# ShijieZhou-UCLA/feature-3dgs

Measured on NVIDIA B200. Metric: views/sec fwd+bwd @1M Gaussians/1080p/feat_dim=128, higher is better.
Workload: dtype f32

## Files before the change

feature-3dgs_b200/csrc/api.cu:

```cuda
#include <cub/cub.cuh>

#include <cstdio>
#include <cstdlib>
#include <cstring>
#include <mutex>
#include <string>
#include <vector>

#include "../../include/f3dgs_b200.h"
#include "kernels.h"

#ifndef F3DGS_FBWD_TC_DEFAULT
#define F3DGS_FBWD_TC_DEFAULT 0
#endif
#ifndef F3DGS_BWD2_DEFAULT
#define F3DGS_BWD2_DEFAULT 1
#endif
#ifndef F3DGS_TC_DEFAULT
#define F3DGS_TC_DEFAULT 1
#endif

namespace f3dgs {
std::atomic<unsigned long long> g_launches{0};
}
// ... 66 lines not shown
    size_t final_T, n_contrib, ranges, counters, bytes;
    ImgLayout(size_t HW, size_t tiles) {
        size_t o = 0;
        final_T = o;    o = align_up(o + HW * 4);
        n_contrib = o;  o = align_up(o + HW * 4);
        ranges = o;     o = align_up(o + tiles * 8);
        counters = o;   o = align_up(o + 256);
        bytes = o;
    }
};
struct BinLayout {
    size_t point_list, keys, point_list_unsorted, keys_unsorted, fixed_bytes;
    explicit BinLayout(size_t R) {
        size_t o = 0;
        point_list = o;           o = align_up(o + R * 4);
        keys = o;                 o = align_up(o + R * 8);
        point_list_unsorted = o;  o = align_up(o + R * 4);
        keys_unsorted = o;        o = align_up(o + R * 8);
        fixed_bytes = o;
    }
};

struct ListLayout {
    size_t w, meta, cnt, bytes;
    ListLayout(size_t R, size_t tiles) {
        size_t o = 0;
        w = o;     o = align_up(o + 8 * R * 32 * sizeof(float));
        meta = o;  o = align_up(o + 8 * R * sizeof(uint2));
        cnt = o;   o = align_up(o + 8 * tiles * sizeof(uint32_t));
        bytes = o;
    }
};

inline bool bwd2_mode() {
    static int on = -1;
    if (on < 0) {
        const char* e = getenv("F3DGS_BWD2");
        on = e ? (e[0] == '1' ? 1 : 0) : F3DGS_BWD2_DEFAULT;
    }
    return on != 0;
}

inline bool tc_mode(int C, const float* features) {
    static int on = -1;
    if (on < 0) {
        const char* e = getenv("F3DGS_TC");
        on = e ? (e[0] == '1' ? 1 : 0) : F3DGS_TC_DEFAULT;
    }
    static int min_c = -1;
    if (min_c < 0) {
        const char* e = getenv("F3DGS_TC_MIN_C");
// ... 292 lines not shown
            char* lists = nullptr;
            const ListLayout ll((size_t)R, tiles);
            if (C > 0 && R > 0) {
                static std::once_flag once;
                std::call_once(once, [] {
                    int dev = 0;
                    cudaGetDevice(&dev);
                    cudaMemPool_t pool;
                    if (cudaDeviceGetDefaultMemPool(&pool, dev) == cudaSuccess) {
                        unsigned long long keep = ~0ull;
                        cudaMemPoolSetAttribute(pool, cudaMemPoolAttrReleaseThreshold, &keep);
                    }
                });
                cudaError_t ea = cudaMallocAsync((void**)&lists, ll.bytes, stream);
                if (ea != cudaSuccess)
                    return fail(F3DGS_ERR_ALLOC, w + ": cudaMallocAsync of " + std::to_string(ll.bytes) +
                                                     " bytes for the backward instance lists failed: " +
                                                     cudaGetErrorString(ea));
            }
            e = launch_composite_bwd_geom_slim(
                vg, ranges, point_list, rec, background, final_T, n_contrib, dL_dpix, dL_depths, dL_dmean2D, dL_dconic,
                dL_dopacity, dL_dcolor, dL_dz, counters + 16, stream, lists ? reinterpret_cast<float*>(lists + ll.w) : nullptr,
                lists ? reinterpret_cast<uint2*>(lists + ll.meta) : nullptr,
                lists ? reinterpret_cast<uint32_t*>(lists + ll.cnt) : nullptr);
            if (e == cudaSuccess && lists)
                e = launch_feature_bwd(vp, ranges, reinterpret_cast<const float*>(lists + ll.w),
                                       reinterpret_cast<const uint2*>(lists + ll.meta),
                                       reinterpret_cast<const uint32_t*>(lists + ll.cnt), dL_dfeaturepix,
                                       dL_dsemantic_feature, counters + 48, stream, fbwd_tc_mode(C));
            if (lists) cudaFreeAsync(lists, stream);
        } else {
            e = launch_composite_bwd(vp, ranges, point_list, rec, background, final_T, n_contrib, dL_dpix,
                                     dL_dfeaturepix, dL_depths, dL_dmean2D, dL_dconic, dL_dopacity, dL_dcolor,
                                     dL_dsemantic_feature, dL_dz, counters + 16, stream);
        }
    }
    if (e != cudaSuccess) return fail(F3DGS_ERR_CUDA, std::string("composite_bwd launch: ") + cudaGetErrorString(e));
    STAGE_CHECK("composite_bwd");
    if (composite_done) CUDA_TRY(cudaEventRecord(composite_done, stream));
    {
        StageTimer t(F3DGS_STAGE_PREPROCESS_BWD, stream);
        launch_preprocess_bwd(vp, means3D, radii, shs, clamped, scales, rotations, cov3d, dL_dmean2D, dL_dconic,
                              dL_dmean3D, dL_dcolor, dL_dcov3D, dL_dsh, dL_dscale, dL_drot, dL_dz, stream, accumulate,
                              grad_accum, denom);
    }
    STAGE_CHECK("preprocess_bwd");
    return 0;
}

}

// ... 102 lines not shown
```

feature-3dgs_b200/csrc/composite_bwd.cu:

```cuda
#include <cstdio>
#include <cstdlib>

#include "composite_common.cuh"

namespace f3dgs {

#ifndef F3DGS_TIMING_BUILD
#define F3DGS_TIMING_BUILD 0
#endif
#ifndef F3DGS_DIAG_NO_FEAT_RED
#define F3DGS_DIAG_NO_FEAT_RED 0
#endif
#ifndef F3DGS_DIAG_NO_FMA
#define F3DGS_DIAG_NO_FMA 0
#endif
#ifndef F3DGS_DIAG_NO_GEOM_RED
#define F3DGS_DIAG_NO_GEOM_RED 0
#endif
static constexpr bool kTimingB = F3DGS_TIMING_BUILD != 0;
#define BTICK() ((kTimingB && args.dbg) ? clock64() : 0ll)

#ifndef F3DGS_PAIR_SKIP
#define F3DGS_PAIR_SKIP 1
#endif
// ... 30 lines not shown
    uint32_t red_gid[kBlocksPerTile][kRedSlots];
};
using BwdSmem = BwdSmemT<RingV2<0>>;

struct BwdArgs {
    ProducerArgs pa;
    const float* bg;
    const float* final_T;
    const uint32_t* n_contrib;
    const float* dL_dpix;
    const float* dL_dfeat_pix;
    const float* dL_ddepth;
    float* dL_dmean2D;
    float* dL_dconic;
    float* dL_dopacity;
    float* dL_dcolor;
    float* dL_dfeature;
    float* dL_dz;
    int vec_io;
    long long* dbg;
    float* list_w;
    uint2* list_meta;
    uint32_t* list_cnt;
};

__device__ __forceinline__ float* geom_dst(const BwdArgs& args, int v, uint32_t gid) {
    switch (v) {
        case 0: return args.dL_dmean2D + 3 * (size_t)gid;
        case 1: return args.dL_dmean2D + 3 * (size_t)gid + 1;
        case 2: return args.dL_dconic + 4 * (size_t)gid;
        case 3: return args.dL_dconic + 4 * (size_t)gid + 1;
        case 4: return args.dL_dconic + 4 * (size_t)gid + 3;
        case 5: return args.dL_dopacity + gid;
        case 6: return args.dL_dz + gid;
        default: return args.dL_dcolor + 3 * (size_t)gid + (v - 7);
    }
}


template <int CH, int BPA, bool SLIM = false, bool EMIT = false>
__global__ void __launch_bounds__(SLIM ? (kAlphaWarp0 + Layout<BPA>::kAlphaWarps) * 32 : Layout<BPA>::kThreads, SLIM ? kSlimCtas : 1)
composite_bwd_kernel(const BwdArgs args) {
    static_assert(!SLIM || CH == 0, "the slim layout has no feature warps");
    extern __shared__ __align__(128) unsigned char smem_raw[];
    using RING = typename RingSelect<0, SLIM>::type;
    using SMEM = BwdSmemT<RING>;
// ... 201 lines not shown
                                const float dL_dG = r1.w * dL_dalpha;
                                const float gdx = Gs * dx, gdy = Gs * dy;
                                const float dG_ddelx = -gdx * r1.x - gdy * r1.y;
                                const float dG_ddely = -gdy * r1.z - gdx * r1.y;
                                v[0] = dL_dG * dG_ddelx * ddelx_dx;
                                v[1] = dL_dG * dG_ddely * ddely_dy;
                                v[2] = -0.5f * gdx * dx * dL_dG;
                                v[3] = -0.5f * gdx * dy * dL_dG;
                                v[4] = -0.5f * gdy * dy * dL_dG;
                                v[5] = Gs * dL_dalpha;
                                v[6] = wgt * p.dLd;
                            }
                            const uint32_t pm = __ballot_sync(0xffffffffu, contrib);
                            if (pm) {
                                if (kTimingB) nA_pm++;
                                if (CH > 0) {
                                    ws->w[k][lane] = wgt;
                                    if (lane == 0) ws->pm[k] = pm;
                                    km |= 1u << k;
                                }
                                if (EMIT) {
                                    const size_t e = ebase[bi] + ecount[bi];
                                    args.list_w[e * 32 + lane] = wgt;
                                    if (lane == 0) args.list_meta[e] = make_uint2(st.gid[k], pm);
                                    ecount[bi]++;
                                }
                                if (do_geom) {
#pragma unroll
                                    for (int i = 0; i < kRedVals; i++) red[i * kRedSlots + nslots][lane] = v[i];
                                    if (lane == 0) red_gid[nslots] = st.gid[k];
                                    nslots++;
                                    if (nslots == kRedSlots) flush();
                                }
                            }
                        }
                    }
                }
                if (CH > 0) {
                    __syncwarp();
                    if (lane == 0) {
                        ws->km = km;
                        ws->last = last;
                        ws->first = first;
                        ws->work = work;
                        mbar_arrive(&ring.wfull[b][j]);
                    }
                }
// ... 231 lines not shown
    g_launches++;
    if (timing) {
        static long long host[256 * 32 * 8];
        cudaMemcpyAsync(host, dbg, sizeof(host), cudaMemcpyDeviceToHost, s);
        cudaStreamSynchronize(s);
        const int nA = Layout<BPA>::kAlphaWarps, f0 = Layout<BPA>::kFeatWarp0;
        double A[6] = {0, 0, 0, 0, 0, 0}, F[6] = {0, 0, 0, 0, 0, 0};
        for (int c = 0; c < grid; c++) {
            for (int w = 0; w < nA; w++) for (int i = 0; i < 6; i++) A[i] += host[(c * 32 + kAlphaWarp0 + w) * 8 + i];
            for (int w = 0; w < 8; w++) for (int i = 0; i < 6; i++) F[i] += host[(c * 32 + f0 + w) * 8 + i];
        }
        fprintf(stderr, "[f3dgs timing bwd CH=%d BPA=%d] per-warp mean cycles: alpha total %.0f wait_full %.0f wait_wempty %.0f flush %.0f hits %.0f pm %.0f | feature total %.0f wait_wfull %.0f wait_full %.0f tile_load %.0f k %.0f k_loop %.0f\n",
                CH, BPA, A[0] / (grid * nA), A[1] / (grid * nA), A[2] / (grid * nA), A[3] / (grid * nA), A[4] / (grid * nA),
                A[5] / (grid * nA), F[0] / (grid * 8), F[1] / (grid * 8), F[2] / (grid * 8), F[3] / (grid * 8), F[4] / (grid * 8), F[5] / (grid * 8));
    }
    return cudaGetLastError();
}

cudaError_t launch_composite_bwd_geom_slim(const ViewParams& vp, const uint2* ranges, const uint32_t* point_list,
                                           const SplatRec* rec, const float* bg, const float* final_T,
                                           const uint32_t* n_contrib, const float* dL_dpix, const float* dL_ddepth,
                                           float* dL_dmean2D, float* dL_dconic, float* dL_dopacity, float* dL_dcolor,
                                           float* dL_dz, int* work_counter, cudaStream_t s, float* list_w,
                                           uint2* list_meta, uint32_t* list_cnt) {
    using SMEM = BwdSmemT<RingSlim>;
    const bool emit = list_w != nullptr;
    const size_t smem = sizeof(SMEM);
    static std::atomic<int> sms_of_device[64];
    int dev = 0;
    cudaGetDevice(&dev);
    if (dev < 0 || dev >= 64) return cudaErrorInvalidDevice;
    if (sms_of_device[dev].load() == 0) {
        cudaError_t e = cudaFuncSetAttribute(composite_bwd_kernel<0, 1, true>, cudaFuncAttributeMaxDynamicSharedMemorySize,
                                             (int)smem);
        if (e == cudaSuccess)
            e = cudaFuncSetAttribute(composite_bwd_kernel<0, 1, true, true>, cudaFuncAttributeMaxDynamicSharedMemorySize,
                                     (int)smem);
        if (e != cudaSuccess) return e;
        int n = 0;
        cudaDeviceGetAttribute(&n, cudaDevAttrMultiProcessorCount, dev);
        sms_of_device[dev].store(n > 0 ? n : 148);
    }
    BwdArgs a;
    a.pa.ranges = ranges; a.pa.point_list = point_list; a.pa.rec = rec; a.pa.features = nullptr;
    a.pa.n_contrib = n_contrib; a.pa.work_counter = work_counter;
    a.pa.W = vp.W; a.pa.H = vp.H; a.pa.C = 0;
    a.pa.tiles_x = (int)vp.grid_x; a.pa.num_tiles = (int)(vp.grid_x * vp.grid_y); a.pa.chunks = 1; a.pa.use_bulk = 0;
    a.bg = bg; a.final_T = final_T; a.n_contrib = n_contrib; a.dL_dpix = dL_dpix; a.dL_dfeat_pix = nullptr;
    a.dL_ddepth = dL_ddepth; a.dL_dmean2D = dL_dmean2D; a.dL_dconic = dL_dconic; a.dL_dopacity = dL_dopacity;
    a.dL_dcolor = dL_dcolor; a.dL_dfeature = nullptr; a.dL_dz = dL_dz; a.vec_io = 0; a.dbg = nullptr;
    a.list_w = list_w; a.list_meta = list_meta; a.list_cnt = list_cnt;
    cudaError_t e = cudaMemsetAsync(work_counter, 0, sizeof(int), s);
    if (e != cudaSuccess) return e;
    const int grid = min(a.pa.num_tiles, kSlimCtas * sms_of_device[dev].load());
    if (emit)
        composite_bwd_kernel<0, 1, true, true><<<grid, (kAlphaWarp0 + Layout<1>::kAlphaWarps) * 32, smem, s>>>(a);
    else
        composite_bwd_kernel<0, 1, true><<<grid, (kAlphaWarp0 + Layout<1>::kAlphaWarps) * 32, smem, s>>>(a);
    g_launches++;
    return cudaGetLastError();
}

#define F3DGS_BWD_DISPATCH(CHV) launch_bwd_t<CHV, 1>(vp, a, s)

cudaError_t launch_composite_bwd(const ViewParams& vp, const uint2* ranges, const uint32_t* point_list,
                                 const SplatRec* rec, const float* bg, const float* final_T,
                                 const uint32_t* n_contrib, const float* dL_dpix, const float* dL_dfeat_pix,
                                 const float* dL_ddepth, float* dL_dmean2D, float* dL_dconic,
                                 float* dL_dopacity, float* dL_dcolor, float* dL_dfeature, float* dL_dz,
                                 int* work_counter, cudaStream_t s) {
    BwdArgs a;
    a.pa.ranges = ranges; a.pa.point_list = point_list; a.pa.rec = rec; a.pa.features = nullptr;
    a.pa.n_contrib = n_contrib; a.pa.work_counter = work_counter;
    a.pa.W = vp.W; a.pa.H = vp.H; a.pa.C = vp.C;
    a.pa.tiles_x = (int)vp.grid_x; a.pa.num_tiles = (int)(vp.grid_x * vp.grid_y); a.pa.chunks = 1;
    a.pa.use_bulk = 0;
    a.bg = bg; a.final_T = final_T; a.n_contrib = n_contrib; a.dL_dpix = dL_dpix; a.dL_dfeat_pix = dL_dfeat_pix;
    a.dL_ddepth = dL_ddepth; a.dL_dmean2D = dL_dmean2D; a.dL_dconic = dL_dconic; a.dL_dopacity = dL_dopacity;
    a.dL_dcolor = dL_dcolor; a.dL_dfeature = dL_dfeature; a.dL_dz = dL_dz; a.vec_io = 0; a.dbg = nullptr;
    a.list_w = nullptr; a.list_meta = nullptr; a.list_cnt = nullptr;
    if (vp.C == 0) return F3DGS_BWD_DISPATCH(0);
    if (vp.C <= 32) return F3DGS_BWD_DISPATCH(32);
    if (vp.C <= 64) return F3DGS_BWD_DISPATCH(64);
    return F3DGS_BWD_DISPATCH(128);
}

}
```

feature-3dgs_b200/csrc/feature_bwd.cu:

```cuda
#include <cstdio>
#include <cstdlib>

#include "composite_common.cuh"
#include "tc_common.cuh"

namespace f3dgs {

#ifndef F3DGS_LIST_CHUNK
#define F3DGS_LIST_CHUNK 16
#endif
constexpr int kListChunk = F3DGS_LIST_CHUNK;
constexpr int kFeatWarps = 4;

template <int CH, bool WITH_ROWS>
struct alignas(128) FeatSmem {
    float w[2][kListChunk][32];
};

struct FeatArgs {
    const uint2* ranges;
    const float* list_w;
    const uint2* list_meta;
    const uint32_t* list_cnt;
    const float* dL_dfeat_pix;
    float* dL_dfeature;
    int* work_counter;
    int W, H, C, tiles_x, num_tiles, chunks;
    int vec;
};

__device__ __forceinline__ void cp_async16(void* dst_smem, const void* src_gmem) {
    asm volatile("cp.async.ca.shared.global [%0], [%1], 16;" ::"r"(smem_u32(dst_smem)), "l"(src_gmem) : "memory");
}
__device__ __forceinline__ void cp_async_commit() { asm volatile("cp.async.commit_group;" ::: "memory"); }
template <int N>
__device__ __forceinline__ void cp_async_wait() {
    asm volatile("cp.async.wait_group %0;" ::"n"(N) : "memory");
}

struct ItemPos {
    int tile, chunk, b, bx0, by0;
};
__device__ __forceinline__ ItemPos decode_item(int item, const FeatArgs& a) {
    ItemPos p;
    p.b = item & (kBlocksPerTile - 1);
    const int tc = item / kBlocksPerTile;
    p.chunk = tc % a.chunks;
    p.tile = tc / a.chunks;
    const int tile_x = p.tile % a.tiles_x, tile_y = p.tile / a.tiles_x;
    p.bx0 = tile_x * 16 + (p.b & 1) * 8;
    p.by0 = tile_y * 16 + (p.b >> 1) * 4;
    return p;
}

template <int CH>
__global__ void __launch_bounds__(kFeatWarps * 32, 3) feature_bwd_kernel(const FeatArgs a) {
    extern __shared__ __align__(128) unsigned char smem_raw[];
    const int warp = __shfl_sync(0xffffffffu, threadIdx.x >> 5, 0), lane = threadIdx.x & 31;
    FeatSmem<CH, false>& sm = reinterpret_cast<FeatSmem<CH, false>*>(smem_raw)[warp];
    constexpr int LPR = CH / 4;
    constexpr int G = 32 / LPR;
    constexpr int NQ = 8 / G;
    const int grp = lane / LPR, cl = lane % LPR;
    const int W = a.W, H = a.H, C = a.C;
    const size_t HW = (size_t)H * W;

    const int items = a.num_tiles * a.chunks * kBlocksPerTile;
    for (;;) {
        int item = 0;
        if (lane == 0) item = atomicAdd(a.work_counter, 1);
        item = __shfl_sync(0xffffffffu, item, 0);
        if (item >= items) break;
        const ItemPos ip = decode_item(item, a);
        const uint32_t rx = __shfl_sync(0xffffffffu, a.ranges[ip.tile].x, 0);
        const uint32_t ry = __shfl_sync(0xffffffffu, a.ranges[ip.tile].y, 0);
        const size_t base = 8 * (size_t)rx + (size_t)ip.b * (ry - rx);
        const uint32_t n = __shfl_sync(0xffffffffu, a.list_cnt[(size_t)ip.tile * kBlocksPerTile + ip.b], 0);
        if (n == 0) continue;
        const int ch0 = ip.chunk * CH + cl * 4;
        const uint32_t nch = (n + kListChunk - 1) / kListChunk;

        auto load_meta = [&](uint32_t c) -> uint2 {
            const uint32_t e = c * kListChunk + lane;
            return (lane < kListChunk && e < n) ? __ldg(&a.list_meta[base + e]) : make_uint2(0u, 0u);
        };
        auto issue = [&](uint32_t c, int buf) {
            const uint32_t cnt = min((uint32_t)kListChunk, n - c * kListChunk);
            const float* wsrc = a.list_w + (base + (size_t)c * kListChunk) * 32;
            for (uint32_t j = lane; j < cnt * 8; j += 32) cp_async16(&sm.w[buf][0][0] + j * 4, wsrc + j * 4);
            cp_async_commit();
        };
        uint2 m_cur = load_meta(0);
        issue(0, 0);

        float2 dO2[NQ][2][4];
#define DOB(q, i, c) (((i) & 1) ? dO2[q][(i) >> 1][c].y : dO2[q][(i) >> 1][c].x)
#pragma unroll
        for (int q = 0; q < NQ; q++)
#pragma unroll
            for (int r = 0; r < 2; r++)
#pragma unroll
                for (int c = 0; c < 4; c++) dO2[q][r][c] = make_float2(0.f, 0.f);
#pragma unroll
        for (int c = 0; c < 4; c++) {
            const int ch = ch0 + c;
            if (ch >= C) continue;
            const float* plane = a.dL_dfeat_pix + (size_t)ch * HW;
            if (G == 1 && (a.vec & 2)) {
#pragma unroll
                for (int y = 0; y < 4; y++) {
                    const int yy = ip.by0 + y;
                    if (yy >= H) continue;
#pragma unroll
                    for (int half = 0; half < 2; half++) {
                        const int xx = ip.bx0 + half * 4;
                        if (xx >= W) continue;
                        const int qa = (y >> 1) * 4 + half * 2, i0 = (y & 1) * 2;
                        const float4 v = ld_nc_f4(plane + (size_t)yy * W + xx);
                        DOB(qa % NQ, i0, c) = v.x;
                        DOB(qa % NQ, i0 + 1, c) = v.y;
                        DOB((qa + 1) % NQ, i0, c) = v.z;
                        DOB((qa + 1) % NQ, i0 + 1, c) = v.w;
                    }
                }
            } else {
#pragma unroll
                for (int qi = 0; qi < NQ; qi++) {
                    const int q = qi * G + grp;
#pragma unroll
                    for (int i = 0; i < 4; i++) {
                        const int xx = ip.bx0 + (q & 3) * 2 + (i & 1), yy = ip.by0 + (q >> 2) * 2 + (i >> 1);
                        if (xx < W && yy < H) DOB(qi, i, c) = __ldg(plane + (size_t)yy * W + xx);
                    }
                }
            }
        }
#undef DOB

        for (uint32_t c = 0; c < nch; c++) {
            const int buf = c & 1;
            const uint2 m_nxt = load_meta(c + 1);
            if (c + 1 < nch) {
                issue(c + 1, buf ^ 1);
                cp_async_wait<1>();
            } else {
                cp_async_wait<0>();
            }
            __syncwarp();
            const uint32_t cnt = min((uint32_t)kListChunk, n - c * kListChunk);
            for (uint32_t i = 0; i < cnt; i++) {
                const uint32_t gid = __shfl_sync(0xffffffffu, m_cur.x, i);
                const uint32_t pm = __shfl_sync(0xffffffffu, m_cur.y, i);
                float2 gp[4];
#pragma unroll
                for (int ch = 0; ch < 4; ch++) gp[ch] = make_float2(0.f, 0.f);
#pragma unroll
                for (int qi = 0; qi < NQ; qi++) {
                    const int q = qi * G + grp;
                    if ((pm >> (4 * q)) & 0xFu) {
                        const float4 w4 = *reinterpret_cast<const float4*>(&sm.w[buf][i][4 * q]);
                        const float2 w01 = make_float2(w4.x, w4.y), w23 = make_float2(w4.z, w4.w);
#pragma unroll
                        for (int ch = 0; ch < 4; ch++) gp[ch] = __ffma2_rn(w01, dO2[qi][0][ch], gp[ch]);
#pragma unroll
                        for (int ch = 0; ch < 4; ch++) gp[ch] = __ffma2_rn(w23, dO2[qi][1][ch], gp[ch]);
                    }
                }
                float g0 = gp[0].x + gp[0].y, g1 = gp[1].x + gp[1].y, g2 = gp[2].x + gp[2].y, g3 = gp[3].x + gp[3].y;
#pragma unroll
                for (int o = LPR; o < 32; o <<= 1) {
                    g0 += __shfl_xor_sync(0xffffffffu, g0, o);
                    g1 += __shfl_xor_sync(0xffffffffu, g1, o);
                    g2 += __shfl_xor_sync(0xffffffffu, g2, o);
                    g3 += __shfl_xor_sync(0xffffffffu, g3, o);
                }
                if (grp == 0 && ch0 < C) {
                    float* dst = a.dL_dfeature + (size_t)gid * C + ch0;
                    if (a.vec & 1) {
                        red_add_f4(dst, make_float4(g0, g1, g2, g3));
                    } else {
                        red_add_f1(dst, g0);
                        if (ch0 + 1 < C) red_add_f1(dst + 1, g1);
                        if (ch0 + 2 < C) red_add_f1(dst + 2, g2);
                        if (ch0 + 3 < C) red_add_f1(dst + 3, g3);
                    }
                }
            }
            __syncwarp();
            m_cur = m_nxt;
        }
    }
}

namespace {

constexpr int kFbHelp0 = 0, kFbLoad0 = 4, kFbLoadWarpsPerGroup = 4, kFbGroups = 2;
constexpr int kFbEpi0 = 12, kFbEpiN = 4;
constexpr int kFbThreads = (kFbEpi0 + kFbEpiN) * 32;
constexpr int kFbRows = 128;
constexpr int kFbTrStride = 132;

struct alignas(1024) FbSlot {
    float Ahi[kFbRows][32];
    float Alo[kFbRows][32];
    float Bhi[128][32];
    float Blo[128][32];
};
static_assert(sizeof(FbSlot) == 64 * 1024, "operand slot is 64 KB");

struct alignas(1024) FbSmem {
    FbSlot slot[kFbGroups];
    float tr[kFbEpiN][32][kFbTrStride];
    uint32_t tr_gid[kFbEpiN][32];
// ... 281 lines not shown
    } else if (helpers) {
        const int ew = warp - kFbHelp0;
        for (;;) {
            pair_sync(ew);
            const int rows = *reinterpret_cast<volatile int32_t*>(&sm.tr_rows[ew]);
            if (rows < 0) break;
            const int ch0 = *reinterpret_cast<volatile int32_t*>(&sm.tr_ch0[ew]);
            fb_reduce_rows(sm, ew, lane, 1, 2, rows, ch0, a);
            __syncwarp();
            pair_sync(ew);
        }
    }

    tc_fence_before();
    __syncthreads();
    if (warp == 0) {
        tc_fence_after();
        tmem_dealloc<256>(tmem);
    }
}

}

static int workers_grid() {
    static std::atomic<int> sms_of_device[64];
    int dev = 0;
    cudaGetDevice(&dev);
    if (dev < 0 || dev >= 64) return 148 * 3;
    if (sms_of_device[dev].load() == 0) {
        int n = 0;
        cudaDeviceGetAttribute(&n, cudaDevAttrMultiProcessorCount, dev);
        sms_of_device[dev].store(n > 0 ? n : 148);
    }
    return sms_of_device[dev].load() * 3;
}

template <int CH>
static cudaError_t launch_feat_bwd_t(const FeatArgs& a, cudaStream_t s) {
    const size_t smem = kFeatWarps * sizeof(FeatSmem<CH, false>);
    const int items = a.num_tiles * a.chunks * kBlocksPerTile;
    const int grid = min((items + kFeatWarps - 1) / kFeatWarps, workers_grid());
    feature_bwd_kernel<CH><<<grid, kFeatWarps * 32, smem, s>>>(a);
    g_launches++;
    return cudaGetLastError();
}

static int feat_ch(int C) { return C <= 32 ? 32 : (C <= 64 ? 64 : 128); }

cudaError_t launch_feature_bwd(const ViewParams& vp, const uint2* ranges, const float* list_w, const uint2* list_meta,
                               const uint32_t* list_cnt, const float* dL_dfeat_pix, float* dL_dfeature,
                               int* work_counter, cudaStream_t s, bool use_tc) {
    FeatArgs a;
    a.ranges = ranges; a.list_w = list_w; a.list_meta = list_meta; a.list_cnt = list_cnt;
    a.dL_dfeat_pix = dL_dfeat_pix; a.dL_dfeature = dL_dfeature;
    a.work_counter = work_counter;
    a.W = vp.W; a.H = vp.H; a.C = vp.C; a.tiles_x = (int)vp.grid_x; a.num_tiles = (int)(vp.grid_x * vp.grid_y);
    const int CH = feat_ch(vp.C);
    a.chunks = (vp.C + CH - 1) / CH;
    a.vec = 0;
    if (vp.C % 4 == 0 && (reinterpret_cast<uintptr_t>(dL_dfeature) & 15) == 0) a.vec |= 1;
    if (vp.W % 4 == 0 && (reinterpret_cast<uintptr_t>(dL_dfeat_pix) & 15) == 0) a.vec |= 2;
    cudaError_t e = cudaMemsetAsync(work_counter, 0, sizeof(int), s);
    if (e != cudaSuccess) return e;
    if (use_tc && (a.vec & 1)) {
        a.chunks = (vp.C + 127) / 128;
        const size_t smem = sizeof(FbSmem) + 1024;
        static std::atomic<int> sms_of_device[64];
        int dev = 0;
        cudaGetDevice(&dev);
        if (dev < 0 || dev >= 64) return cudaErrorInvalidDevice;
        if (sms_of_device[dev].load() == 0) {
            e = cudaFuncSetAttribute(feature_bwd_tc_kernel, cudaFuncAttributeMaxDynamicSharedMemorySize, (int)smem);
            if (e != cudaSuccess) return e;
            int n = 0;
            cudaDeviceGetAttribute(&n, cudaDevAttrMultiProcessorCount, dev);
            sms_of_device[dev].store(n > 0 ? n : 148);
// ... 4 lines not shown
                const char* e = getenv(name);
                return (e ? atoi(e) : dflt) != 0;
            };
            return (on("F3DGS_FBTC_HELPERS", 1) ? kFbHelpers : 0) | (on("F3DGS_FBTC_DIAG", 0) ? kFbDiag : 0) |
                   (on("F3DGS_FBTC_PREFETCH", 1) ? kFbPrefetch : 0);
        }();
        const int grid = min(items, sms_of_device[dev].load());
        feature_bwd_tc_kernel<<<grid, kFbThreads, smem, s>>>(a, flags);
        g_launches++;
        e = cudaGetLastError();
        if (e == cudaSuccess && (flags & kFbDiag)) {
            unsigned long long d[8] = {0};
            const unsigned long long zero[8] = {0};
            cudaStreamSynchronize(s);
            cudaMemcpyFromSymbol(d, fbtc_diag, sizeof(d));
            cudaMemcpyToSymbol(fbtc_diag, zero, sizeof(zero));
            fprintf(stderr, "fbtc_diag: loader0 loop %.0f wait_slot %.0f handovers %.1f | epi0 loop %.0f wait_acc %.0f drain %.0f (cycles per CTA, %d CTAs)\n",
                    (double)d[0] / grid, (double)d[1] / grid, (double)d[2] / grid, (double)d[3] / grid, (double)d[4] / grid,
                    (double)d[5] / grid, grid);
        }
        return e;
    }
    if (CH == 32) return launch_feat_bwd_t<32>(a, s);
    if (CH == 64) return launch_feat_bwd_t<64>(a, s);
    return launch_feat_bwd_t<128>(a, s);
}

}
```

feature-3dgs_b200/csrc/kernels.h:

```cpp
#pragma once
#include <cuda_runtime.h>
#include <stdint.h>

#include <atomic>

#include "common.cuh"

namespace f3dgs {

extern std::atomic<unsigned long long> g_launches;

struct ViewParams {
    int P, D, M, C;
    int W, H;
    uint32_t grid_x, grid_y;
    float tan_fovx, tan_fovy, focal_x, focal_y;
    float scale_modifier;
    const float* viewmatrix;
    const float* projmatrix;
    const float* cam_pos;
};

void launch_preprocess_fwd(const ViewParams& vp, const float* means3D, const float* scales,
                           const float* rotations, const float* opacities, const float* shs,
// ... 11 lines not shown
void launch_mark_visible(int P, const float* means3D, const float* viewmatrix, uint8_t* present,
                         cudaStream_t s);

void launch_duplicate_keys(int P, const SplatRec* rec, const uint32_t* offsets, const int* radii,
                           uint32_t grid_x, uint32_t grid_y, uint64_t* keys, uint32_t* values,
                           cudaStream_t s);
void launch_tile_ranges(int R, const uint64_t* sorted_keys, uint2* ranges, cudaStream_t s);

cudaError_t launch_composite_fwd(const ViewParams& vp, const uint2* ranges, const uint32_t* point_list,
                                 const SplatRec* rec, const float* features, const float* bg,
                                 float* final_T, uint32_t* n_contrib, float* out_color,
                                 float* out_feature, float* out_depth, int* work_counter, cudaStream_t s);

cudaError_t launch_composite_fwd_tc(const ViewParams& vp, const uint2* ranges, const uint32_t* point_list,
                                    const SplatRec* rec, const float* features, const float* bg,
                                    float* final_T, uint32_t* n_contrib, float* out_color,
                                    float* out_feature, float* out_depth, int* work_counter, cudaStream_t s);

cudaError_t launch_composite_bwd_geom_slim(const ViewParams& vp, const uint2* ranges, const uint32_t* point_list,
                                           const SplatRec* rec, const float* bg, const float* final_T,
                                           const uint32_t* n_contrib, const float* dL_dpix, const float* dL_ddepth,
                                           float* dL_dmean2D, float* dL_dconic, float* dL_dopacity, float* dL_dcolor,
                                           float* dL_dz, int* work_counter, cudaStream_t s, float* list_w = nullptr,
                                           uint2* list_meta = nullptr, uint32_t* list_cnt = nullptr);

cudaError_t launch_feature_bwd(const ViewParams& vp, const uint2* ranges, const float* list_w, const uint2* list_meta,
                               const uint32_t* list_cnt, const float* dL_dfeat_pix, float* dL_dfeature,
                               int* work_counter, cudaStream_t s, bool use_tc = false);

cudaError_t launch_composite_bwd(const ViewParams& vp, const uint2* ranges, const uint32_t* point_list,
                                 const SplatRec* rec, const float* bg, const float* final_T,
                                 const uint32_t* n_contrib, const float* dL_dpix, const float* dL_dfeat_pix,
                                 const float* dL_ddepth, float* dL_dmean2D, float* dL_dconic,
                                 float* dL_dopacity, float* dL_dcolor, float* dL_dfeature, float* dL_dz,
                                 int* work_counter, cudaStream_t s);

cudaError_t launch_feature_resize_fwd(int C, int H, int W, int Hg, int Wg, const float* fm, const float* gt,
                                      float grad_scale, float* out, float* loss_sum, cudaStream_t s);
cudaError_t launch_feature_resize_bwd(int C, int H, int W, int Hg, int Wg, const float* dout, float* dfm, cudaStream_t s);

}
```

feature-3dgs_b200/csrc/preprocess.cu:

```cuda
#include <cstdio>

#include "kernels.h"

namespace f3dgs {

__device__ __constant__ float kSH_C0 = 0.28209479177387814f;
__device__ __constant__ float kSH_C1 = 0.4886025119029199f;
__device__ __constant__ float kSH_C2[5] = {1.0925484305920792f, -1.0925484305920792f, 0.31539156525252005f,
                                           -1.0925484305920792f, 0.5462742152960396f};
__device__ __constant__ float kSH_C3[7] = {-0.5900435899266435f, 2.890611442640554f, -0.4570457994644658f,
                                           0.3731763325901154f,  -0.4570457994644658f, 1.445305721320277f,
                                           -0.5900435899266435f};

struct F3 {
    float x, y, z;
};
__device__ __forceinline__ F3 operator+(F3 a, F3 b) { return F3{a.x + b.x, a.y + b.y, a.z + b.z}; }
__device__ __forceinline__ F3 operator-(F3 a, F3 b) { return F3{a.x - b.x, a.y - b.y, a.z - b.z}; }
__device__ __forceinline__ F3 operator*(float s, F3 a) { return F3{s * a.x, s * a.y, s * a.z}; }
__device__ __forceinline__ F3 operator/(F3 a, float s) { return F3{a.x / s, a.y / s, a.z / s}; }

struct M3 {
    float c[3][3];
};
// ... 485 lines not shown
#pragma unroll
            for (int rr = 0; rr < 3; rr++)
                dM[cc][rr] = 2.0f * (M[0][rr] * S[cc][0] + M[1][rr] * S[cc][1] + M[2][rr] * S[cc][2]);
        float dMt[3][3];
#pragma unroll
        for (int cc = 0; cc < 3; cc++)
#pragma unroll
            for (int rr = 0; rr < 3; rr++) dMt[cc][rr] = dM[rr][cc];
#pragma unroll
        for (int k = 0; k < 3; k++)
            put<ACCUM>(dL_dscale + 3 * idx + k, R[0][k] * dMt[k][0] + R[1][k] * dMt[k][1] + R[2][k] * dMt[k][2]);
#pragma unroll
        for (int k = 0; k < 3; k++)
#pragma unroll
            for (int rr = 0; rr < 3; rr++) dMt[k][rr] *= s[k];
        float4 dq;
        dq.x = 2 * z * (dMt[0][1] - dMt[1][0]) + 2 * y * (dMt[2][0] - dMt[0][2]) + 2 * x * (dMt[1][2] - dMt[2][1]);
        dq.y = 2 * y * (dMt[1][0] + dMt[0][1]) + 2 * z * (dMt[2][0] + dMt[0][2]) + 2 * r * (dMt[1][2] - dMt[2][1]) -
               4 * x * (dMt[2][2] + dMt[1][1]);
        dq.z = 2 * x * (dMt[1][0] + dMt[0][1]) + 2 * r * (dMt[2][0] - dMt[0][2]) + 2 * z * (dMt[1][2] + dMt[2][1]) -
               4 * y * (dMt[2][2] + dMt[0][0]);
        dq.w = 2 * r * (dMt[0][1] - dMt[1][0]) + 2 * x * (dMt[2][0] + dMt[0][2]) + 2 * y * (dMt[1][2] + dMt[2][1]) -
               4 * z * (dMt[1][1] + dMt[0][0]);
        if (ACCUM) {
            const float4 o = reinterpret_cast<float4*>(dL_drot)[idx];
            dq.x += o.x; dq.y += o.y; dq.z += o.z; dq.w += o.w;
        }
        reinterpret_cast<float4*>(dL_drot)[idx] = dq;
    }
    }
    if (shs != nullptr) {
        __syncthreads();
        float* dst = dL_dsh + (size_t)block_base * row_floats;
        if ((row_floats & 3) == 0 && (reinterpret_cast<uintptr_t>(dL_dsh) & 15) == 0) {
            const int q_per_row = row_floats >> 2;
            for (int i = threadIdx.x; i < rows_here * q_per_row; i += kBwdBlock) {
                const int row = i / q_per_row;
                if (!vis[row]) continue;
                const float* g = dsh_rows + row * stride + (i % q_per_row) * 4;
                float4 v = make_float4(g[0], g[1], g[2], g[3]);
                float4* o = reinterpret_cast<float4*>(dst) + i;
                if (ACCUM) {
                    const float4 old = *o;
                    v.x += old.x; v.y += old.y; v.z += old.z; v.w += old.w;
                }
                *o = v;
            }
        } else {
            for (int i = threadIdx.x; i < rows_here * row_floats; i += kBwdBlock) {
                const int row = i / row_floats;
                if (!vis[row]) continue;
// ... 58 lines not shown
```

Measured before the change: 197.6.

## Merge paired block instance lists in feature backward to share atomic reductions

The geometry backward now also emits each instance's list position. The feature backward gives each warp a pair of adjacent 8x4 pixel blocks and walks their two lists in lockstep by position. When both blocks hold the same Gaussian, their contributions are summed before a single red.add to the feature gradient, which cuts global atomics and lets one work item cover two blocks. Metadata and positions are now staged through cp.async into shared memory. The cost is more registers (two sets of dO), a smaller channel chunk (64 instead of 128 for C=128), an extra list buffer, and an alignment fallback added to the dL_drot store.

```diff
diff --git a/feature-3dgs_b200/csrc/api.cu b/feature-3dgs_b200/csrc/api.cu
--- a/feature-3dgs_b200/csrc/api.cu
+++ b/feature-3dgs_b200/csrc/api.cu
@@ -112,11 +112,12 @@
 };
 
 struct ListLayout {
-    size_t w, meta, cnt, bytes;
+    size_t w, meta, pos, cnt, bytes;
     ListLayout(size_t R, size_t tiles) {
         size_t o = 0;
         w = o;     o = align_up(o + 8 * R * 32 * sizeof(float));
         meta = o;  o = align_up(o + 8 * R * sizeof(uint2));
+        pos = o;   o = align_up(o + 8 * R * sizeof(uint32_t));
         cnt = o;   o = align_up(o + 8 * tiles * sizeof(uint32_t));
         bytes = o;
     }
@@ -455,11 +456,13 @@
                 vg, ranges, point_list, rec, background, final_T, n_contrib, dL_dpix, dL_depths, dL_dmean2D, dL_dconic,
                 dL_dopacity, dL_dcolor, dL_dz, counters + 16, stream, lists ? reinterpret_cast<float*>(lists + ll.w) : nullptr,
                 lists ? reinterpret_cast<uint2*>(lists + ll.meta) : nullptr,
-                lists ? reinterpret_cast<uint32_t*>(lists + ll.cnt) : nullptr);
+                lists ? reinterpret_cast<uint32_t*>(lists + ll.cnt) : nullptr,
+                lists ? reinterpret_cast<uint32_t*>(lists + ll.pos) : nullptr);
             if (e == cudaSuccess && lists)
                 e = launch_feature_bwd(vp, ranges, reinterpret_cast<const float*>(lists + ll.w),
                                        reinterpret_cast<const uint2*>(lists + ll.meta),
-                                       reinterpret_cast<const uint32_t*>(lists + ll.cnt), dL_dfeaturepix,
+                                       reinterpret_cast<const uint32_t*>(lists + ll.cnt),
+                                       reinterpret_cast<const uint32_t*>(lists + ll.pos), dL_dfeaturepix,
                                        dL_dsemantic_feature, counters + 48, stream, fbwd_tc_mode(C));
             if (lists) cudaFreeAsync(lists, stream);
         } else {
diff --git a/feature-3dgs_b200/csrc/composite_bwd.cu b/feature-3dgs_b200/csrc/composite_bwd.cu
--- a/feature-3dgs_b200/csrc/composite_bwd.cu
+++ b/feature-3dgs_b200/csrc/composite_bwd.cu
@@ -76,6 +76,7 @@
     float* list_w;
     uint2* list_meta;
     uint32_t* list_cnt;
+    uint32_t* list_pos;
 };
 
 __device__ __forceinline__ float* geom_dst(const BwdArgs& args, int v, uint32_t gid) {
@@ -323,7 +324,10 @@
                                 if (EMIT) {
                                     const size_t e = ebase[bi] + ecount[bi];
                                     args.list_w[e * 32 + lane] = wgt;
-                                    if (lane == 0) args.list_meta[e] = make_uint2(st.gid[k], pm);
+                                    if (lane == 0) {
+                                        args.list_meta[e] = make_uint2(st.gid[k], pm);
+                                        args.list_pos[e] = st.listpos[k];
+                                    }
                                     ecount[bi]++;
                                 }
                                 if (do_geom) {
@@ -601,7 +605,7 @@
                                            const uint32_t* n_contrib, const float* dL_dpix, const float* dL_ddepth,
                                            float* dL_dmean2D, float* dL_dconic, float* dL_dopacity, float* dL_dcolor,
                                            float* dL_dz, int* work_counter, cudaStream_t s, float* list_w,
-                                           uint2* list_meta, uint32_t* list_cnt) {
+                                           uint2* list_meta, uint32_t* list_cnt, uint32_t* list_pos) {
     using SMEM = BwdSmemT<RingSlim>;
     const bool emit = list_w != nullptr;
     const size_t smem = sizeof(SMEM);
@@ -628,7 +632,7 @@
     a.bg = bg; a.final_T = final_T; a.n_contrib = n_contrib; a.dL_dpix = dL_dpix; a.dL_dfeat_pix = nullptr;
     a.dL_ddepth = dL_ddepth; a.dL_dmean2D = dL_dmean2D; a.dL_dconic = dL_dconic; a.dL_dopacity = dL_dopacity;
     a.dL_dcolor = dL_dcolor; a.dL_dfeature = nullptr; a.dL_dz = dL_dz; a.vec_io = 0; a.dbg = nullptr;
-    a.list_w = list_w; a.list_meta = list_meta; a.list_cnt = list_cnt;
+    a.list_w = list_w; a.list_meta = list_meta; a.list_cnt = list_cnt; a.list_pos = list_pos;
     cudaError_t e = cudaMemsetAsync(work_counter, 0, sizeof(int), s);
     if (e != cudaSuccess) return e;
     const int grid = min(a.pa.num_tiles, kSlimCtas * sms_of_device[dev].load());
@@ -657,7 +661,7 @@
     a.bg = bg; a.final_T = final_T; a.n_contrib = n_contrib; a.dL_dpix = dL_dpix; a.dL_dfeat_pix = dL_dfeat_pix;
     a.dL_ddepth = dL_ddepth; a.dL_dmean2D = dL_dmean2D; a.dL_dconic = dL_dconic; a.dL_dopacity = dL_dopacity;
     a.dL_dcolor = dL_dcolor; a.dL_dfeature = dL_dfeature; a.dL_dz = dL_dz; a.vec_io = 0; a.dbg = nullptr;
-    a.list_w = nullptr; a.list_meta = nullptr; a.list_cnt = nullptr;
+    a.list_w = nullptr; a.list_meta = nullptr; a.list_cnt = nullptr; a.list_pos = nullptr;
     if (vp.C == 0) return F3DGS_BWD_DISPATCH(0);
     if (vp.C <= 32) return F3DGS_BWD_DISPATCH(32);
     if (vp.C <= 64) return F3DGS_BWD_DISPATCH(64);
diff --git a/feature-3dgs_b200/csrc/feature_bwd.cu b/feature-3dgs_b200/csrc/feature_bwd.cu
--- a/feature-3dgs_b200/csrc/feature_bwd.cu
+++ b/feature-3dgs_b200/csrc/feature_bwd.cu
@@ -11,10 +11,12 @@
 #endif
 constexpr int kListChunk = F3DGS_LIST_CHUNK;
 constexpr int kFeatWarps = 4;
-
-template <int CH, bool WITH_ROWS>
+constexpr int kPairsPerTile = kBlocksPerTile / 2;
+
 struct alignas(128) FeatSmem {
-    float w[2][kListChunk][32];
+    float w[2][2][kListChunk][32];
+    uint2 meta[2][2][kListChunk];
+    uint32_t pos[2][2][kListChunk];
 };
 
 struct FeatArgs {
@@ -22,6 +24,7 @@
     const float* list_w;
     const uint2* list_meta;
     const uint32_t* list_cnt;
+    const uint32_t* list_pos;
     const float* dL_dfeat_pix;
     float* dL_dfeature;
     int* work_counter;
@@ -29,8 +32,9 @@
     int vec;
 };
 
-__device__ __forceinline__ void cp_async16(void* dst_smem, const void* src_gmem) {
-    asm volatile("cp.async.ca.shared.global [%0], [%1], 16;" ::"r"(smem_u32(dst_smem)), "l"(src_gmem) : "memory");
+template <int BYTES = 16>
+__device__ __forceinline__ void cp_async(void* dst_smem, const void* src_gmem) {
+    asm volatile("cp.async.ca.shared.global [%0], [%1], %2;" ::"r"(smem_u32(dst_smem)), "l"(src_gmem), "n"(BYTES) : "memory");
 }
 __device__ __forceinline__ void cp_async_commit() { asm volatile("cp.async.commit_group;" ::: "memory"); }
 template <int N>
@@ -57,7 +61,7 @@
 __global__ void __launch_bounds__(kFeatWarps * 32, 3) feature_bwd_kernel(const FeatArgs a) {
     extern __shared__ __align__(128) unsigned char smem_raw[];
     const int warp = __shfl_sync(0xffffffffu, threadIdx.x >> 5, 0), lane = threadIdx.x & 31;
-    FeatSmem<CH, false>& sm = reinterpret_cast<FeatSmem<CH, false>*>(smem_raw)[warp];
+    FeatSmem& sm = reinterpret_cast<FeatSmem*>(smem_raw)[warp];
     constexpr int LPR = CH / 4;
     constexpr int G = 32 / LPR;
     constexpr int NQ = 8 / G;
@@ -65,130 +69,169 @@
     const int W = a.W, H = a.H, C = a.C;
     const size_t HW = (size_t)H * W;
 
-    const int items = a.num_tiles * a.chunks * kBlocksPerTile;
+    const int items = a.num_tiles * a.chunks * kPairsPerTile;
     for (;;) {
         int item = 0;
         if (lane == 0) item = atomicAdd(a.work_counter, 1);
         item = __shfl_sync(0xffffffffu, item, 0);
         if (item >= items) break;
-        const ItemPos ip = decode_item(item, a);
-        const uint32_t rx = __shfl_sync(0xffffffffu, a.ranges[ip.tile].x, 0);
-        const uint32_t ry = __shfl_sync(0xffffffffu, a.ranges[ip.tile].y, 0);
-        const size_t base = 8 * (size_t)rx + (size_t)ip.b * (ry - rx);
-        const uint32_t n = __shfl_sync(0xffffffffu, a.list_cnt[(size_t)ip.tile * kBlocksPerTile + ip.b], 0);
-        if (n == 0) continue;
-        const int ch0 = ip.chunk * CH + cl * 4;
-        const uint32_t nch = (n + kListChunk - 1) / kListChunk;
-
-        auto load_meta = [&](uint32_t c) -> uint2 {
-            const uint32_t e = c * kListChunk + lane;
-            return (lane < kListChunk && e < n) ? __ldg(&a.list_meta[base + e]) : make_uint2(0u, 0u);
-        };
-        auto issue = [&](uint32_t c, int buf) {
-            const uint32_t cnt = min((uint32_t)kListChunk, n - c * kListChunk);
-            const float* wsrc = a.list_w + (base + (size_t)c * kListChunk) * 32;
-            for (uint32_t j = lane; j < cnt * 8; j += 32) cp_async16(&sm.w[buf][0][0] + j * 4, wsrc + j * 4);
+        const int pair = item % kPairsPerTile;
+        const int tc = item / kPairsPerTile;
+        const int chunk = tc % a.chunks, tile = tc / a.chunks;
+        const int bx0 = (tile % a.tiles_x) * 16, by0 = (tile / a.tiles_x) * 16 + pair * 4;
+        const uint32_t rx = __shfl_sync(0xffffffffu, a.ranges[tile].x, 0);
+        const uint32_t ry = __shfl_sync(0xffffffffu, a.ranges[tile].y, 0);
+        size_t base[2];
+        uint32_t n[2], nch[2];
+#pragma unroll
+        for (int h = 0; h < 2; h++) {
+            const int b = 2 * pair + h;
+            base[h] = 8 * (size_t)rx + (size_t)b * (ry - rx);
+            n[h] = __shfl_sync(0xffffffffu, a.list_cnt[(size_t)tile * kBlocksPerTile + b], 0);
+            nch[h] = (n[h] + kListChunk - 1) / kListChunk;
+        }
+        if (n[0] == 0 && n[1] == 0) continue;
+        const int ch0 = chunk * CH + cl * 4;
+
+        auto issue = [&](int h, uint32_t c) {
+            if (c < nch[h]) {
+                const uint32_t cnt = min((uint32_t)kListChunk, n[h] - c * kListChunk);
+                const size_t e0 = base[h] + (size_t)c * kListChunk;
+                const float* wsrc = a.list_w + e0 * 32;
+                for (uint32_t j = lane; j < cnt * 8; j += 32) cp_async(&sm.w[h][c & 1][0][0] + j * 4, wsrc + j * 4);
+                if ((uint32_t)lane < cnt) {
+                    cp_async<8>(&sm.meta[h][c & 1][lane], a.list_meta + e0 + lane);
+                    cp_async<4>(&sm.pos[h][c & 1][lane], a.list_pos + e0 + lane);
+                }
+            }
             cp_async_commit();
         };
-        uint2 m_cur = load_meta(0);
         issue(0, 0);
-
-        float2 dO2[NQ][2][4];
-#define DOB(q, i, c) (((i) & 1) ? dO2[q][(i) >> 1][c].y : dO2[q][(i) >> 1][c].x)
-#pragma unroll
-        for (int q = 0; q < NQ; q++)
-#pragma unroll
-            for (int r = 0; r < 2; r++)
-#pragma unroll
-                for (int c = 0; c < 4; c++) dO2[q][r][c] = make_float2(0.f, 0.f);
+        issue(1, 0);
+        issue(0, 1);
+        issue(1, 1);
+
+        float2 dO2[2][NQ][2][4];
+#define DOB(h, q, i, c) (((i) & 1) ? dO2[h][q][(i) >> 1][c].y : dO2[h][q][(i) >> 1][c].x)
+#pragma unroll
+        for (int h = 0; h < 2; h++)
+#pragma unroll
+            for (int q = 0; q < NQ; q++)
+#pragma unroll
+                for (int r = 0; r < 2; r++)
+#pragma unroll
+                    for (int c = 0; c < 4; c++) dO2[h][q][r][c] = make_float2(0.f, 0.f);
 #pragma unroll
         for (int c = 0; c < 4; c++) {
             const int ch = ch0 + c;
             if (ch >= C) continue;
             const float* plane = a.dL_dfeat_pix + (size_t)ch * HW;
-            if (G == 1 && (a.vec & 2)) {
-#pragma unroll
-                for (int y = 0; y < 4; y++) {
-                    const int yy = ip.by0 + y;
-                    if (yy >= H) continue;
-#pragma unroll
-                    for (int half = 0; half < 2; half++) {
-                        const int xx = ip.bx0 + half * 4;
-                        if (xx >= W) continue;
-                        const int qa = (y >> 1) * 4 + half * 2, i0 = (y & 1) * 2;
-                        const float4 v = ld_nc_f4(plane + (size_t)yy * W + xx);
-                        DOB(qa % NQ, i0, c) = v.x;
-                        DOB(qa % NQ, i0 + 1, c) = v.y;
-                        DOB((qa + 1) % NQ, i0, c) = v.z;
-                        DOB((qa + 1) % NQ, i0 + 1, c) = v.w;
+#pragma unroll
+            for (int h = 0; h < 2; h++) {
+                const int hx0 = bx0 + h * 8;
+                if (G == 1 && (a.vec & 2)) {
+#pragma unroll
+                    for (int y = 0; y < 4; y++) {
+                        const int yy = by0 + y;
+                        if (yy >= H) continue;
+#pragma unroll
+                        for (int half = 0; half < 2; half++) {
+                            const int xx = hx0 + half * 4;
+                            if (xx >= W) continue;
+                            const int qa = (y >> 1) * 4 + half * 2, i0 = (y & 1) * 2;
+                            const float4 v = ld_nc_f4(plane + (size_t)yy * W + xx);
+                            DOB(h, qa % NQ, i0, c) = v.x;
+                            DOB(h, qa % NQ, i0 + 1, c) = v.y;
+                            DOB(h, (qa + 1) % NQ, i0, c) = v.z;
+                            DOB(h, (qa + 1) % NQ, i0 + 1, c) = v.w;
+                        }
                     }
-                }
-            } else {
-#pragma unroll
-                for (int qi = 0; qi < NQ; qi++) {
-                    const int q = qi * G + grp;
-#pragma unroll
-                    for (int i = 0; i < 4; i++) {
-                        const int xx = ip.bx0 + (q & 3) * 2 + (i & 1), yy = ip.by0 + (q >> 2) * 2 + (i >> 1);
-                        if (xx < W && yy < H) DOB(qi, i, c) = __ldg(plane + (size_t)yy * W + xx);
+                } else {
+#pragma unroll
+                    for (int qi = 0; qi < NQ; qi++) {
+                        const int q = qi * G + grp;
+#pragma unroll
+                        for (int i = 0; i < 4; i++) {
+                            const int xx = hx0 + (q & 3) * 2 + (i & 1), yy = by0 + (q >> 2) * 2 + (i >> 1);
+                            if (xx < W && yy < H) DOB(h, qi, i, c) = __ldg(plane + (size_t)yy * W + xx);
+                        }
                     }
                 }
             }
         }
 #undef DOB
 
-        for (uint32_t c = 0; c < nch; c++) {
-            const int buf = c & 1;
-            const uint2 m_nxt = load_meta(c + 1);
-            if (c + 1 < nch) {
-                issue(c + 1, buf ^ 1);
-                cp_async_wait<1>();
-            } else {
-                cp_async_wait<0>();
-            }
-            __syncwarp();
-            const uint32_t cnt = min((uint32_t)kListChunk, n - c * kListChunk);
-            for (uint32_t i = 0; i < cnt; i++) {
-                const uint32_t gid = __shfl_sync(0xffffffffu, m_cur.x, i);
-                const uint32_t pm = __shfl_sync(0xffffffffu, m_cur.y, i);
-                float2 gp[4];
-#pragma unroll
-                for (int ch = 0; ch < 4; ch++) gp[ch] = make_float2(0.f, 0.f);
+        cp_async_wait<2>();
+        __syncwarp();
+        uint32_t e[2] = {0u, 0u};
+        while (e[0] < n[0] || e[1] < n[1]) {
+            uint32_t p[2];
+            uint2 m[2];
+#pragma unroll
+            for (int h = 0; h < 2; h++) {
+                const uint32_t s = (e[h] / kListChunk) & 1, i = e[h] % kListChunk;
+                p[h] = e[h] < n[h] ? sm.pos[h][s][i] : 0u;
+                m[h] = sm.meta[h][s][i];
+            }
+            const bool take0 = p[0] >= p[1], take1 = p[1] >= p[0];
+            const uint32_t gid = take0 ? m[0].x : m[1].x;
+            float2 gp[4];
+#pragma unroll
+            for (int ch = 0; ch < 4; ch++) gp[ch] = make_float2(0.f, 0.f);
+#pragma unroll
+            for (int h = 0; h < 2; h++) {
+                const bool take = h == 0 ? take0 : take1;
+                if (!take) continue;
+                const uint32_t pm = m[h].y;
+                const float* wrow = &sm.w[h][(e[h] / kListChunk) & 1][e[h] % kListChunk][0];
 #pragma unroll
                 for (int qi = 0; qi < NQ; qi++) {
                     const int q = qi * G + grp;
                     if ((pm >> (4 * q)) & 0xFu) {
-                        const float4 w4 = *reinterpret_cast<const float4*>(&sm.w[buf][i][4 * q]);
+                        const float4 w4 = *reinterpret_cast<const float4*>(wrow + 4 * q);
                         const float2 w01 = make_float2(w4.x, w4.y), w23 = make_float2(w4.z, w4.w);
 #pragma unroll
-                        for (int ch = 0; ch < 4; ch++) gp[ch] = __ffma2_rn(w01, dO2[qi][0][ch], gp[ch]);
-#pragma unroll
-                        for (int ch = 0; ch < 4; ch++) gp[ch] = __ffma2_rn(w23, dO2[qi][1][ch], gp[ch]);
+                        for (int ch = 0; ch < 4; ch++) gp[ch] = __ffma2_rn(w01, dO2[h][qi][0][ch], gp[ch]);
+#pragma unroll
+                        for (int ch = 0; ch < 4; ch++) gp[ch] = __ffma2_rn(w23, dO2[h][qi][1][ch], gp[ch]);
                     }
                 }
-                float g0 = gp[0].x + gp[0].y, g1 = gp[1].x + gp[1].y, g2 = gp[2].x + gp[2].y, g3 = gp[3].x + gp[3].y;
-#pragma unroll
-                for (int o = LPR; o < 32; o <<= 1) {
-                    g0 += __shfl_xor_sync(0xffffffffu, g0, o);
-                    g1 += __shfl_xor_sync(0xffffffffu, g1, o);
-                    g2 += __shfl_xor_sync(0xffffffffu, g2, o);
-                    g3 += __shfl_xor_sync(0xffffffffu, g3, o);
-                }
-                if (grp == 0 && ch0 < C) {
-                    float* dst = a.dL_dfeature + (size_t)gid * C + ch0;
-                    if (a.vec & 1) {
-                        red_add_f4(dst, make_float4(g0, g1, g2, g3));
-                    } else {
-                        red_add_f1(dst, g0);
-                        if (ch0 + 1 < C) red_add_f1(dst + 1, g1);
-                        if (ch0 + 2 < C) red_add_f1(dst + 2, g2);
-                        if (ch0 + 3 < C) red_add_f1(dst + 3, g3);
-                    }
-                }
-            }
-            __syncwarp();
-            m_cur = m_nxt;
-        }
+            }
+            float g0 = gp[0].x + gp[0].y, g1 = gp[1].x + gp[1].y, g2 = gp[2].x + gp[2].y, g3 = gp[3].x + gp[3].y;
+#pragma unroll
+            for (int o = LPR; o < 32; o <<= 1) {
+                g0 += __shfl_xor_sync(0xffffffffu, g0, o);
+                g1 += __shfl_xor_sync(0xffffffffu, g1, o);
+                g2 += __shfl_xor_sync(0xffffffffu, g2, o);
+                g3 += __shfl_xor_sync(0xffffffffu, g3, o);
+            }
+            if (grp == 0 && ch0 < C) {
+                float* dst = a.dL_dfeature + (size_t)gid * C + ch0;
+                if (a.vec & 1) {
+                    red_add_f4(dst, make_float4(g0, g1, g2, g3));
+                } else {
+                    red_add_f1(dst, g0);
+                    if (ch0 + 1 < C) red_add_f1(dst + 1, g1);
+                    if (ch0 + 2 < C) red_add_f1(dst + 2, g2);
+                    if (ch0 + 3 < C) red_add_f1(dst + 3, g3);
+                }
+            }
+#pragma unroll
+            for (int h = 0; h < 2; h++) {
+                const bool take = h == 0 ? take0 : take1;
+                if (!take) continue;
+                e[h]++;
+                if (e[h] % kListChunk == 0 && e[h] < n[h]) {
+                    const uint32_t c = e[h] / kListChunk;
+                    __syncwarp();
+                    issue(h, c + 1);
+                    cp_async_wait<1>();
+                    __syncwarp();
+                }
+            }
+        }
+        cp_async_wait<0>();
+        __syncwarp();
     }
 }
 
@@ -516,36 +559,36 @@
 
 }
 
-static int workers_grid() {
+static int sm_count() {
     static std::atomic<int> sms_of_device[64];
     int dev = 0;
     cudaGetDevice(&dev);
-    if (dev < 0 || dev >= 64) return 148 * 3;
+    if (dev < 0 || dev >= 64) return 148;
     if (sms_of_device[dev].load() == 0) {
         int n = 0;
         cudaDeviceGetAttribute(&n, cudaDevAttrMultiProcessorCount, dev);
         sms_of_device[dev].store(n > 0 ? n : 148);
     }
-    return sms_of_device[dev].load() * 3;
+    return sms_of_device[dev].load();
 }
 
 template <int CH>
 static cudaError_t launch_feat_bwd_t(const FeatArgs& a, cudaStream_t s) {
-    const size_t smem = kFeatWarps * sizeof(FeatSmem<CH, false>);
-    const int items = a.num_tiles * a.chunks * kBlocksPerTile;
-    const int grid = min((items + kFeatWarps - 1) / kFeatWarps, workers_grid());
+    const size_t smem = kFeatWarps * sizeof(FeatSmem);
+    const int items = a.num_tiles * a.chunks * kPairsPerTile;
+    const int grid = min((items + kFeatWarps - 1) / kFeatWarps, sm_count() * 3);
     feature_bwd_kernel<CH><<<grid, kFeatWarps * 32, smem, s>>>(a);
     g_launches++;
     return cudaGetLastError();
 }
 
-static int feat_ch(int C) { return C <= 32 ? 32 : (C <= 64 ? 64 : 128); }
+static int feat_ch(int C) { return C <= 32 ? 32 : 64; }
 
 cudaError_t launch_feature_bwd(const ViewParams& vp, const uint2* ranges, const float* list_w, const uint2* list_meta,
-                               const uint32_t* list_cnt, const float* dL_dfeat_pix, float* dL_dfeature,
-                               int* work_counter, cudaStream_t s, bool use_tc) {
+                               const uint32_t* list_cnt, const uint32_t* list_pos, const float* dL_dfeat_pix,
+                               float* dL_dfeature, int* work_counter, cudaStream_t s, bool use_tc) {
     FeatArgs a;
-    a.ranges = ranges; a.list_w = list_w; a.list_meta = list_meta; a.list_cnt = list_cnt;
+    a.ranges = ranges; a.list_w = list_w; a.list_meta = list_meta; a.list_cnt = list_cnt; a.list_pos = list_pos;
     a.dL_dfeat_pix = dL_dfeat_pix; a.dL_dfeature = dL_dfeature;
     a.work_counter = work_counter;
     a.W = vp.W; a.H = vp.H; a.C = vp.C; a.tiles_x = (int)vp.grid_x; a.num_tiles = (int)(vp.grid_x * vp.grid_y);
@@ -596,8 +639,7 @@
         return e;
     }
     if (CH == 32) return launch_feat_bwd_t<32>(a, s);
-    if (CH == 64) return launch_feat_bwd_t<64>(a, s);
-    return launch_feat_bwd_t<128>(a, s);
-}
-
-}
+    return launch_feat_bwd_t<64>(a, s);
+}
+
+}
diff --git a/feature-3dgs_b200/csrc/kernels.h b/feature-3dgs_b200/csrc/kernels.h
--- a/feature-3dgs_b200/csrc/kernels.h
+++ b/feature-3dgs_b200/csrc/kernels.h
@@ -57,11 +57,12 @@
                                            const uint32_t* n_contrib, const float* dL_dpix, const float* dL_ddepth,
                                            float* dL_dmean2D, float* dL_dconic, float* dL_dopacity, float* dL_dcolor,
                                            float* dL_dz, int* work_counter, cudaStream_t s, float* list_w = nullptr,
-                                           uint2* list_meta = nullptr, uint32_t* list_cnt = nullptr);
+                                           uint2* list_meta = nullptr, uint32_t* list_cnt = nullptr,
+                                           uint32_t* list_pos = nullptr);
 
 cudaError_t launch_feature_bwd(const ViewParams& vp, const uint2* ranges, const float* list_w, const uint2* list_meta,
-                               const uint32_t* list_cnt, const float* dL_dfeat_pix, float* dL_dfeature,
-                               int* work_counter, cudaStream_t s, bool use_tc = false);
+                               const uint32_t* list_cnt, const uint32_t* list_pos, const float* dL_dfeat_pix,
+                               float* dL_dfeature, int* work_counter, cudaStream_t s, bool use_tc = false);
 
 cudaError_t launch_composite_bwd(const ViewParams& vp, const uint2* ranges, const uint32_t* point_list,
                                  const SplatRec* rec, const float* bg, const float* final_T,
diff --git a/feature-3dgs_b200/csrc/preprocess.cu b/feature-3dgs_b200/csrc/preprocess.cu
--- a/feature-3dgs_b200/csrc/preprocess.cu
+++ b/feature-3dgs_b200/csrc/preprocess.cu
@@ -531,11 +531,18 @@
                4 * y * (dMt[2][2] + dMt[0][0]);
         dq.w = 2 * r * (dMt[0][1] - dMt[1][0]) + 2 * x * (dMt[2][0] + dMt[0][2]) + 2 * y * (dMt[1][2] + dMt[2][1]) -
                4 * z * (dMt[1][1] + dMt[0][0]);
-        if (ACCUM) {
-            const float4 o = reinterpret_cast<float4*>(dL_drot)[idx];
-            dq.x += o.x; dq.y += o.y; dq.z += o.z; dq.w += o.w;
-        }
-        reinterpret_cast<float4*>(dL_drot)[idx] = dq;
+        if ((reinterpret_cast<uintptr_t>(dL_drot) & 15) == 0) {
+            if (ACCUM) {
+                const float4 o = reinterpret_cast<float4*>(dL_drot)[idx];
+                dq.x += o.x; dq.y += o.y; dq.z += o.z; dq.w += o.w;
+            }
+            reinterpret_cast<float4*>(dL_drot)[idx] = dq;
+        } else {
+            put<ACCUM>(dL_drot + 4 * idx, dq.x);
+            put<ACCUM>(dL_drot + 4 * idx + 1, dq.y);
+            put<ACCUM>(dL_drot + 4 * idx + 2, dq.z);
+            put<ACCUM>(dL_drot + 4 * idx + 3, dq.w);
+        }
     }
     }
     if (shs != nullptr) {
```

Measured after the change: 168.1 (median of 6 runs). -14.9%, worse.
